# sikang/mpl_ros

Hardware: AMD Instinct MI355X
Metric: node_expansions_per_s (higher is better)
Workload: dtype f64

## Files before the change

include/mplx.h:

```cpp
#ifndef MPLX_H
#define MPLX_H
#include <stdint.h>

#ifdef __cplusplus
extern "C" {
#endif

#define MPLX_OK 0
#define MPLX_ERR_HIP (-1)
#define MPLX_ERR_ARG (-2)
#define MPLX_ERR_CAPACITY (-3)
#define MPLX_ERR_TIMEOUT (-4)

#define MPLX_PLAN_OK 0
#define MPLX_PLAN_NO_PATH 1
#define MPLX_PLAN_START_OCCUPIED 2
#define MPLX_PLAN_MAX_EXPAND 3
#define MPLX_PLAN_POOL_FULL 4
#define MPLX_PLAN_INTERNAL 5
#define MPLX_PLAN_TRAJ_TOO_LONG 6
#define MPLX_PLAN_ABORTED 7

#define MPLX_VEL 1
#define MPLX_ACC 3
// ... 226 lines not shown
int mplx_plpa_result_entries(mplx_plpa *l, uint64_t cap, int32_t *child, int32_t *parent, int32_t *action, int32_t *blocked);
typedef struct mplx_plpa_fleet mplx_plpa_fleet;
int mplx_plpa_fleet_create(mplx_poly *p, int32_t n, const int32_t *world_of, mplx_plpa_fleet **out);
void mplx_plpa_fleet_destroy(mplx_plpa_fleet *f);
const char *mplx_plpa_fleet_last_error(const mplx_plpa_fleet *f);
int mplx_plpa_fleet_size(const mplx_plpa_fleet *f);
mplx_plpa *mplx_plpa_fleet_member(mplx_plpa_fleet *f, int32_t i);
int mplx_plpa_fleet_set_capacity(mplx_plpa_fleet *f, uint64_t nodes, uint64_t edges, uint64_t open_log);
int mplx_plpa_fleet_set_world(mplx_plpa_fleet *f, int32_t i, int32_t world);
int mplx_plpa_fleet_plan(mplx_plpa_fleet *f, const double *starts, const double *goals, const int32_t *active, double eps, double tol_pos, double tol_vel,
                         int32_t max_expand, int32_t heur_ignore_dynamics, mplx_result *out);
int mplx_plpa_fleet_update_nodes(mplx_plpa_fleet *f, uint64_t *n_blocked, uint64_t *n_cleared);
int mplx_plpa_fleet_sub_state_space(mplx_plpa_fleet *f, const int32_t *time_step);
int mplx_plpa_fleet_stats(const mplx_plpa_fleet *f, uint32_t stats[4]);
int mplx_plpa_fleet_last_kernel_ms(const mplx_plpa_fleet *f, float *plan_ms, float *update_ms);
int mplx_poly_last_helpers(const mplx_poly *p);
int mplx_poly_set_deadline(mplx_poly *p, double seconds);
int mplx_poly_result_cycles(mplx_poly *p, int32_t q, uint64_t cyc[10]);

int mplx_result_timing(mplx_ctx *ctx, int q, double *t_begin_s, double *t_end_s, int32_t *slot);
int mplx_result_cycles(mplx_ctx *ctx, int q, uint64_t cyc[10]);
int mplx_result_speculation(mplx_ctx *ctx, int q, uint64_t spec[4]);
int mplx_result_open_dropped(mplx_ctx *ctx, int q, uint64_t *n_dropped);
int mplx_last_kernel_ms(const mplx_ctx *ctx, float *ms);
const char *mplx_kernel_name(const mplx_ctx *ctx);
uint64_t mplx_plan_epoch(const mplx_ctx *ctx);
const char *mplx_version(void);

typedef struct mplx_cloud mplx_cloud;
typedef struct {
  double state[13];
  double cost;
  int32_t action;
  int32_t valid;
} mplx_cloud_succ;
int mplx_cloud_create(int device, mplx_cloud **out);
void mplx_cloud_destroy(mplx_cloud *c);
const char *mplx_cloud_last_error(const mplx_cloud *c);
int mplx_cloud_config(mplx_cloud *c, int32_t control, int32_t n_u, const double *U, double dt, double v_max, double a_max, double j_max, double w);
int mplx_cloud_set_map(mplx_cloud *c, int32_t n, const double *pts, double r, const double ori[3], const double dim[3]);
int mplx_cloud_get_succ_batch(mplx_cloud *c, int32_t K, const double *states, mplx_cloud_succ *out);
uint64_t mplx_cloud_last_point_tests(const mplx_cloud *c);
int mplx_cloud_set_capacity(mplx_cloud *c, int32_t n_slots, uint64_t total_nodes, uint64_t total_edges, uint64_t total_open_log);
int mplx_cloud_plan_batch(mplx_cloud *c, int32_t n, const double *starts, const double *goals, double eps, double tol_pos, double tol_vel,
                          double tol_acc, int32_t max_expand, int32_t heur_ignore_dynamics, mplx_result *out);
int mplx_cloud_result_traj(mplx_cloud *c, int32_t q, mplx_waypoint *wps, int32_t *actions, int32_t *node_ids);
// ... 43 lines not shown
```

mpl_ros_amd/_capi.py:

```python
import ctypes as C
import os

_HERE = os.path.dirname(os.path.abspath(__file__))
LIB_PATH = os.environ.get("MPLX_LIB") or os.path.join(_HERE, "csrc", "libmplx.so")

VEL, ACC, JRK, SNP = 1, 3, 7, 15
PLAN_OK, PLAN_NO_PATH, PLAN_START_OCCUPIED, PLAN_MAX_EXPAND, PLAN_POOL_FULL, PLAN_INTERNAL, PLAN_TRAJ_TOO_LONG = 0, 1, 2, 3, 4, 5, 6
OK, ERR_HIP, ERR_ARG, ERR_CAPACITY, ERR_TIMEOUT = 0, -1, -2, -3, -4


class Waypoint(C.Structure):
    _fields_ = [("pos", C.c_double * 3), ("vel", C.c_double * 3), ("acc", C.c_double * 3),
                ("jrk", C.c_double * 3), ("yaw", C.c_double), ("t", C.c_double),
                ("control", C.c_int32), ("enable_t", C.c_int32)]


class Primitive(C.Structure):
    _fields_ = [("c", (C.c_double * 6) * 3), ("t", C.c_double), ("control", C.c_int32), ("pad", C.c_int32),
                ("cyaw", C.c_double * 6)]


class Config(C.Structure):
    _fields_ = [("control", C.c_int32), ("n_u", C.c_int32), ("U", C.POINTER(C.c_double)),
                ("dt", C.c_double), ("v_max", C.c_double), ("a_max", C.c_double), ("j_max", C.c_double),
# ... 8 lines not shown
                ("key", C.c_int32 * 12), ("nkey", C.c_int32), ("voxel_reads", C.c_int32)]


class Result(C.Structure):
    _fields_ = [("status", C.c_int32), ("traj_len", C.c_int32), ("cost", C.c_double)] + \
               [(n, C.c_uint64) for n in ("n_expanded", "n_closed", "n_nodes", "n_edges", "n_primitives", "n_succ",
                                          "n_succ_finite", "voxel_reads", "n_push", "n_reopen", "n_refill", "n_evict",
                                          "expand_hash")]

    def as_dict(self):
        return {n: getattr(self, n) for n, _ in self._fields_}


class CloudSucc(C.Structure):
    _fields_ = [("state", C.c_double * 13), ("cost", C.c_double), ("action", C.c_int32), ("valid", C.c_int32)]


EXPORTS = [
    "mplx_ctx_create", "mplx_ctx_destroy", "mplx_last_error", "mplx_set_stream",
    "mplx_map_set", "mplx_map_set_device", "mplx_map_free_unknown", "mplx_map_get", "mplx_map_info", "mplx_map_query",
    "mplx_map_dilate", "mplx_map_cells", "mplx_map_raytrace", "mplx_map_cloud",
    "mplx_planner_config", "mplx_set_capacity", "mplx_set_bucket_width", "mplx_set_speculation", "mplx_set_helpers", "mplx_helper_stats",
    "mplx_expand_batch", "mplx_heuristic_batch", "mplx_plan", "mplx_plan_batch",
    "mplx_result_traj", "mplx_set_record", "mplx_result_expanded", "mplx_result_nodes", "mplx_result_edges", "mplx_result_blocked", "mplx_result_timing", "mplx_result_cycles", "mplx_result_speculation", "mplx_result_open_dropped",
    "mplx_last_kernel_ms", "mplx_version", "mplx_kernel_name", "mplx_plan_epoch",
    "mplx_grid_create", "mplx_grid_destroy", "mplx_grid_last_error", "mplx_grid_allocate", "mplx_grid_info", "mplx_grid_clear",
    "mplx_grid_add_cloud", "mplx_grid_add_cloud_inflate", "mplx_grid_decay", "mplx_grid_clear_column", "mplx_grid_fill_column",
    "mplx_grid_fill_cell", "mplx_grid_get_map", "mplx_grid_get_cloud", "mplx_grid_to_map",
    "mplx_potential_weights", "mplx_potential_update", "mplx_search_region_set", "mplx_potential_clear", "mplx_aux_get", "mplx_aux_cloud", "mplx_aux_token",
    "mplx_lpa_create", "mplx_lpa_destroy", "mplx_lpa_last_error", "mplx_lpa_set_capacity", "mplx_lpa_set_record", "mplx_lpa_plan", "mplx_lpa_initialized",
    "mplx_lpa_reset", "mplx_lpa_update_blocked", "mplx_lpa_update_cleared", "mplx_lpa_sub_state_space", "mplx_lpa_set_reroot", "mplx_lpa_traj_len", "mplx_lpa_result_traj",
    "mplx_lpa_counts", "mplx_lpa_result_nodes", "mplx_lpa_result_edges", "mplx_lpa_result_expanded", "mplx_lpa_last_kernel_ms",
    "mplx_lpa_fleet_create", "mplx_lpa_fleet_destroy", "mplx_lpa_fleet_last_error", "mplx_lpa_fleet_size", "mplx_lpa_fleet_member", "mplx_lpa_fleet_set_capacity",
    "mplx_lpa_fleet_plan", "mplx_lpa_fleet_update_blocked", "mplx_lpa_fleet_update_cleared", "mplx_lpa_fleet_sub_state_space", "mplx_lpa_fleet_stats",
    "mplx_lpa_fleet_last_kernel_ms",
    "mplx_poly_create", "mplx_poly_destroy", "mplx_poly_last_error", "mplx_poly_config", "mplx_poly_begin", "mplx_poly_set_world",
    "mplx_poly_add_static", "mplx_poly_add_linear", "mplx_poly_add_nonlinear", "mplx_poly_commit", "mplx_poly_get_succ_batch", "mplx_poly_set_capacity", "mplx_poly_plan_batch", "mplx_poly_result_traj",
    "mplx_poly_set_record", "mplx_poly_result_expanded", "mplx_poly_last_kernel_ms", "mplx_poly_result_cycles", "mplx_poly_set_helpers", "mplx_poly_last_helpers", "mplx_poly_set_deadline", "mplx_plpa_create", "mplx_plpa_destroy", "mplx_plpa_last_error", "mplx_plpa_set_capacity", "mplx_plpa_initialized", "mplx_plpa_reset",
    "mplx_plpa_plan", "mplx_plpa_update_nodes", "mplx_plpa_changed", "mplx_plpa_sub_state_space", "mplx_plpa_traj_len", "mplx_plpa_result_traj", "mplx_plpa_last_kernel_ms", "mplx_plpa_result_cycles",
    "mplx_plpa_counts", "mplx_plpa_result_expanded", "mplx_plpa_result_nodes", "mplx_plpa_result_entries",
    "mplx_plpa_fleet_create", "mplx_plpa_fleet_destroy", "mplx_plpa_fleet_last_error", "mplx_plpa_fleet_size", "mplx_plpa_fleet_member", "mplx_plpa_fleet_set_capacity",
    "mplx_plpa_fleet_set_world", "mplx_plpa_fleet_plan", "mplx_plpa_fleet_update_nodes", "mplx_plpa_fleet_sub_state_space", "mplx_plpa_fleet_stats",
    "mplx_plpa_fleet_last_kernel_ms",
    "mplx_traj_solve", "mplx_traj_sample", "mplx_traj_effort",
    "mplx_plan_batch_submit", "mplx_plan_batch_wait", "mplx_plan_batch_done", "mplx_set_helper_limit", "mplx_release_pools",
    "mplx_set_deadline", "mplx_set_pool_recycling", "mplx_debug_hang_next_launch", "mplx_debug_query_records",
    "mplx_stream_create", "mplx_stream_destroy", "mplx_stream_last_error", "mplx_stream_depth", "mplx_stream_configure",
# ... 49 lines not shown
    L.mplx_map_cells.argtypes = [P, C.c_int, C.c_void_p, C.c_void_p]
    L.mplx_map_raytrace.argtypes = [P, D3, D3, C.c_void_p, C.c_int, C.POINTER(C.c_int)]
    L.mplx_map_cloud.argtypes = [P, C.c_int, C.c_void_p, C.c_uint64, C.POINTER(C.c_uint64)]
    L.mplx_planner_config.argtypes = [P, C.POINTER(Config)]
    L.mplx_set_capacity.argtypes = [P, C.c_int32, C.c_uint64, C.c_uint64, C.c_uint64]
    L.mplx_set_bucket_width.argtypes = [P, C.c_double]
    L.mplx_set_speculation.argtypes = [P, C.c_int32]
    L.mplx_set_helpers.argtypes = [P, C.c_int32, C.c_int32, C.c_uint64]
    L.mplx_helper_stats.argtypes = [P, C.POINTER(C.c_uint32)]
    L.mplx_expand_batch.argtypes = [P, C.c_int, C.POINTER(Waypoint), C.POINTER(Succ)]
    L.mplx_heuristic_batch.argtypes = [P, C.c_int, C.POINTER(Waypoint), C.POINTER(Waypoint), C.c_void_p, C.c_void_p]
    L.mplx_plan.argtypes = [P, C.POINTER(Waypoint), C.POINTER(Waypoint), C.POINTER(Result)]
    L.mplx_plan_batch.argtypes = [P, C.c_int, C.POINTER(Waypoint), C.POINTER(Waypoint), C.POINTER(Result)]
    L.mplx_result_traj.argtypes = [P, C.c_int, C.POINTER(Primitive), C.POINTER(Waypoint), I3, I3]
    L.mplx_set_record.argtypes = [P, C.c_uint32]
    L.mplx_result_expanded.argtypes = [P, C.c_int, C.c_uint32, C.c_void_p, C.POINTER(C.c_uint32)]
    L.mplx_result_nodes.argtypes = [P, C.c_uint64, C.POINTER(Waypoint), C.c_void_p, C.c_void_p, C.c_void_p, C.c_void_p]
    L.mplx_result_edges.argtypes = [P, C.c_void_p, C.c_void_p, C.c_void_p, C.c_uint64, C.POINTER(C.c_uint64)]
    L.mplx_result_blocked.argtypes = [P, C.c_void_p, C.c_void_p, C.c_uint64, C.POINTER(C.c_uint64), C.POINTER(C.c_uint64)]
    L.mplx_result_timing.argtypes = [P, C.c_int, C.POINTER(C.c_double), C.POINTER(C.c_double), I3]
    L.mplx_result_cycles.argtypes = [P, C.c_int, C.POINTER(C.c_uint64)]
    L.mplx_result_speculation.argtypes = [P, C.c_int, C.POINTER(C.c_uint64)]
    L.mplx_result_open_dropped.argtypes = [P, C.c_int, C.POINTER(C.c_uint64)]
    L.mplx_last_kernel_ms.argtypes = [P, C.POINTER(C.c_float)]
    L.mplx_version.restype = C.c_char_p
    L.mplx_kernel_name.argtypes = [P]
    L.mplx_kernel_name.restype = C.c_char_p
    L.mplx_plan_epoch.argtypes = [P]
    L.mplx_plan_epoch.restype = C.c_uint64
    L.mplx_traj_solve.argtypes = [C.c_int32, C.c_int32, C.POINTER(Waypoint), D3, C.POINTER(Primitive)]
    L.mplx_traj_sample.argtypes = [C.c_int32, C.POINTER(Primitive), C.c_int32, C.POINTER(Waypoint), C.c_void_p]
    L.mplx_traj_effort.argtypes = [C.c_int32, C.POINTER(Primitive), C.c_int32]
    L.mplx_traj_effort.restype = C.c_double
    U64 = C.POINTER(C.c_uint64)
    L.mplx_potential_weights.argtypes = [P, C.c_double, C.c_double]
    L.mplx_potential_update.argtypes = [P, D3, D3, D3, C.c_int32]
    L.mplx_search_region_set.argtypes = [P, C.c_int, C.c_void_p, D3, C.c_int]
    L.mplx_potential_clear.argtypes = [P]
    L.mplx_aux_get.argtypes = [P, C.c_void_p]
    L.mplx_aux_token.argtypes = [P, C.c_uint64, C.c_int32, U64]
    L.mplx_aux_cloud.argtypes = [P, C.c_int, C.c_void_p, C.c_void_p, C.c_uint64, U64]
    L.mplx_lpa_create.argtypes = [P, C.POINTER(P)]
    L.mplx_lpa_destroy.argtypes = [P]
    L.mplx_lpa_destroy.restype = None
    L.mplx_lpa_last_error.argtypes = [P]
    L.mplx_lpa_last_error.restype = C.c_char_p
# ... 171 lines not shown
```

mpl_ros_amd/csrc/mplx_api.hip:

```cpp
#include "../../include/mplx.h"

#include <hip/hip_runtime.h>

#include <sched.h>
#include <unistd.h>

#include <algorithm>
#include <chrono>
#include <cmath>
#include <cstdarg>
#include <cstdio>
#include <cstring>
#include <string>
#include <vector>

#define MPLX_UTILITY_KERNELS
#include "mplx_kernels.h"
#include "mplx_poly_dev.h"

using namespace mplx;

static_assert(sizeof(SuccOut) == sizeof(mplx_succ), "SuccOut must mirror mplx_succ");
static_assert(sizeof(State) == 12 * sizeof(double), "State layout");

static std::string g_create_error;

struct mplx_ctx {
  int device = 0;
  hipStream_t stream = nullptr;
  bool own_stream = true;
  std::string err;
  int8_t *map = nullptr;
  bool own_map = false;
  uint32_t *bricks = nullptr;
  int8_t *aux = nullptr;
  double pot_weight = 0.0;
  uint64_t aux_token = 0;
  int32_t dim[3] = {0, 0, 0};
  double origin[3] = {0, 0, 0};
  double res = 0;
// ... 11 lines not shown
  int helpers = -1;
  int help_reserved = -1;
  uint64_t help_rows = 0;
  int n_cus = 0;
  int pool_help_lanes = 0;
  int32_t n_slots = 1;
  uint64_t cap_nodes = 1u << 20, cap_edges = 1u << 22, cap_log = 1u << 21;
  uint32_t cap_rec = 0;
  bool pools_valid = false;
  int32_t pool_slots = 0, pool_control = 0;
  uint64_t pool_nodes = 0, pool_edges = 0, pool_log = 0;
  SearchParams pools{};
  std::vector<void *> pool_allocs;
  std::vector<uint32_t> last_node_table;
  int last_nq = 0;
  bool last_single = false;
  int last_control = 0;
  double last_dt = 0;
  std::vector<double> last_U;
  uint64_t plan_epoch = 0;
  bool help_cache_filled = false;
  uint64_t map_epoch = 0, last_map_epoch = 0;
  std::vector<QueryOut> last_out;
  QueryOut *d_out = nullptr;
  QueryIn *d_in = nullptr;
  int32_t *d_traj_nodes = nullptr, *d_traj_actions = nullptr, *d_rec = nullptr, *d_next = nullptr, *d_order = nullptr;
  uint32_t *d_node_tables = nullptr, *d_edge_tables = nullptr;
  double *d_traj_states = nullptr;
  int batch_cap = 0;
  uint32_t batch_rec = 0;
  hipEvent_t ev0 = nullptr, ev1 = nullptr;
  float last_ms = 0;
  uint32_t help_epoch = 0;
  unsigned long long help_done_init = 0;
  HelpBox *dbg_boxes = nullptr;
  uint32_t help_stats[4] = {0, 0, 0, 0};
  uint32_t help_ctr_back[HELP_CTR_WORDS] = {};
  bool help_stats_pending = false;
  bool pending = false;
  int pend_nq = 0;
  bool pend_help = false;
  std::vector<QueryIn> pend_in;
  std::vector<int32_t> pend_order;
  bool recycle = false;
  uint32_t *d_chunk_bits = nullptr;
  std::vector<uint32_t> chunk_bits_init;
// ... 875 lines not shown
    uint32_t *ctr = nullptr;
    PA(ctr, HELP_CTR_WORDS);
    P.cache_next = ctr;
    P.done_word = (unsigned long long *)(ctr + 32);
    P.cache_rows = (uint32_t)rows;
  }
#undef PA
  P.node_chunks = (uint32_t)nch;
  P.edge_chunks = (uint32_t)ech;
  P.open_chunks = (uint32_t)och;
  P.table_mask = T - 1;
  c->pool_slots = slots;
  c->pool_control = control;
  c->pool_nodes = c->cap_nodes;
  c->pool_edges = c->cap_edges;
  c->pool_log = c->cap_log;
  c->pools_valid = true;
  return MPLX_OK;
}

static int ensure_batch(mplx_ctx *c, int nq) {
  if (c->batch_cap >= nq && c->batch_rec == c->cap_rec) return MPLX_OK;
  free_batch(c);
  HIPCHK(c, hipMalloc((void **)&c->d_out, sizeof(QueryOut) * nq));
  HIPCHK(c, hipMalloc((void **)&c->d_in, sizeof(QueryIn) * nq));
  HIPCHK(c, hipMalloc((void **)&c->d_traj_nodes, sizeof(int32_t) * (size_t)nq * (MAX_TRAJ + 1)));
  HIPCHK(c, hipMalloc((void **)&c->d_traj_actions, sizeof(int32_t) * (size_t)nq * MAX_TRAJ));
  HIPCHK(c, hipMalloc((void **)&c->d_traj_states, sizeof(double) * (size_t)nq * (MAX_TRAJ + 1) * 13));
  HIPCHK(c, hipMalloc((void **)&c->d_traj_yaw, sizeof(double) * (size_t)nq * (MAX_TRAJ + 1)));
  HIPCHK(c, hipMalloc((void **)&c->d_next, sizeof(int32_t)));
  HIPCHK(c, hipMalloc((void **)&c->d_order, sizeof(int32_t) * nq));
  HIPCHK(c, hipMalloc((void **)&c->d_node_tables, sizeof(uint32_t) * (size_t)nq * MAX_NODE_CH));
  HIPCHK(c, hipMalloc((void **)&c->d_edge_tables, sizeof(uint32_t) * (size_t)nq * MAX_EDGE_CH));
  if (c->cap_rec) HIPCHK(c, hipMalloc((void **)&c->d_rec, sizeof(int32_t) * (size_t)nq * c->cap_rec));
  c->batch_cap = nq;
  c->batch_rec = c->cap_rec;
  return MPLX_OK;
}

static void wp_to_state(const mplx_waypoint &w, State &s) {
  for (int i = 0; i < 3; i++) {
    s.p[i] = w.pos[i];
    s.v[i] = (w.control & 2) ? w.vel[i] : 0.0;
    s.a[i] = (w.control & 4) ? w.acc[i] : 0.0;
    s.j[i] = (w.control & 8) ? w.jrk[i] : 0.0;
  }
}
// ... 180 lines not shown
  }
  SearchParams P = c->pools;
  fill_params(c, P, (c->speculation < 0 || c->speculation > 1) && (c->cfg.control == CTRL_ACC || c->cfg.control == CTRL_JRK) && c->cfg.n_u <= 128);
  if (c->wedged) return fail(c, MPLX_ERR_TIMEOUT, "this context was lost to a launch that never ended (destroy it)");
  const int xflags = getenv("MPLX_X_FLAGS") ? atoi(getenv("MPLX_X_FLAGS")) : 0;
  P.xflags = xflags | (c->debug_hang ? 8 : 0);
  c->debug_hang = false;
  guard_arm(c);
  P.cap_rec = c->cap_rec;
  P.nq = nq;
  P.queries = c->d_in;
  P.order = c->d_order;
  P.out = c->d_out;
  P.traj_nodes = c->d_traj_nodes; P.traj_actions = c->d_traj_actions; P.traj_states = c->d_traj_states;
  P.traj_yaw = c->d_traj_yaw;
  P.rec_ids = c->cap_rec ? c->d_rec : nullptr;
  P.node_tables = c->d_node_tables;
  P.edge_tables = c->d_edge_tables;
  P.next_query = c->d_next;
  if (c->filter_table) filter_set(P, c->filter_table, c->filter_mask, c->filter_pool, c->filter_flag);
  HIPCHK(c, hipMemcpyAsync(c->d_order, order.data(), sizeof(int32_t) * nq, hipMemcpyHostToDevice, c->stream));
  if (int rt = table_prepare(c, P, c->stream)) return rt;
  HIPCHK(c, hipMemsetAsync(P.chunk_next, 0, 4 * sizeof(uint32_t), c->stream));
  P.chunk_bits = nullptr;
  HIPCHK(c, hipMemcpyAsync(c->d_in, in.data(), sizeof(QueryIn) * nq, hipMemcpyHostToDevice, c->stream));
  HIPCHK(c, hipMemsetAsync(c->d_next, 0, sizeof(int32_t), c->stream));
  const bool spec = (c->speculation < 0 || c->speculation > 1) && !c->yaw;
  const bool recycle = c->recycle && nq > 1 && spec && !c->filter_table && (P.control == CTRL_ACC || P.control == CTRL_JRK) && P.n_u <= 128 && c->d_chunk_bits;
  if (recycle) {
    HIPCHK(c, hipMemcpyAsync(c->d_chunk_bits, c->chunk_bits_init.data(), sizeof(uint32_t) * c->chunk_bits_init.size(), hipMemcpyHostToDevice, c->stream));
    P.chunk_bits = c->d_chunk_bits;
    for (int k = 0; k < 3; k++) { P.chunk_word0[k] = c->chunk_word0[k]; P.chunk_words[k] = c->chunk_words[k]; }
  }
  c->last_recycled = recycle;
  const int n_wg = c->n_cus;
  int grid = slots;
  P.help_lead = slots;
  P.help_max = 0;
  P.help_limit = c->help_limit;
  const bool help = spec && !c->aux && !c->filter_table && (c->speculation < 0 || c->speculation >= 16) && c->helpers != 0 && P.boxes &&
                    ((P.n_u <= 31 && (P.control == CTRL_ACC || P.control == CTRL_JRK)) || (P.control == CTRL_JRK && P.n_u > 64 && P.n_u <= 128));
  if (help) {
    P.help_max = c->helpers < 0 ? (P.n_u <= 31 ? 4 : 2) : c->helpers;
    P.help_lead = std::min(slots, n_wg);
    const bool long_queries = P.max_expand <= 0 || P.max_expand >= 200000;
    const int reserved = c->help_reserved >= 0 ? c->help_reserved : (nq >= 2 * c->n_cus && long_queries ? std::max(1, c->n_cus / 16) * P.help_max : 0);
// ... 48 lines not shown
}

static int plan_batch_finish(mplx_ctx *c, mplx_result *out) {
  if (!c->pending) return fail(c, MPLX_ERR_ARG, "no submitted batch on this context");
  HIPCHK(c, hipSetDevice(c->device));
  const int nq = c->pend_nq;
  c->pending = false;
  {
    const int rw = guard_wait(c, c->stream, "the search launch");
    if (rw) {
      c->last_nq = 0;
      return rw;
    }
  }
  if (c->pend_help) {
    HIPCHK(c, hipMemcpyAsync(c->help_ctr_back, c->pools.cache_next, HELP_CTR_WORDS * sizeof(uint32_t), hipMemcpyDeviceToHost, c->stream));
    c->help_stats_pending = true;
  } else {
    memset(c->help_stats, 0, sizeof(c->help_stats));
    c->help_stats_pending = false;
  }
  c->last_out.resize(nq);
  HIPCHK(c, hipMemcpyAsync(c->last_out.data(), c->d_out, sizeof(QueryOut) * nq, hipMemcpyDeviceToHost, c->stream));
  HIPCHK(c, hipStreamSynchronize(c->stream));
  HIPCHK(c, hipEventElapsedTime(&c->last_ms, c->ev0, c->ev1));
  if (out)
    for (int i = 0; i < nq; i++) fill_result(c->last_out[i], out[i]);
  c->last_nq = nq;
  c->last_single = (nq == 1);
  c->last_control = c->cfg.control;
  c->last_dt = c->cfg.dt;
  c->last_U = c->U;
  c->last_yaw = c->yaw;
  c->last_Uyaw = c->Uyaw;
  c->last_map_epoch = c->map_epoch;
  c->plan_epoch++;
  return MPLX_OK;
}

extern "C" int mplx_plan_batch(mplx_ctx *c, int nq, const mplx_waypoint *starts, const mplx_waypoint *goals, mplx_result *out) {
  if (!out) return fail(c, MPLX_ERR_ARG, "bad argument");
  int r = plan_batch_launch(c, nq, starts, goals);
  if (r) return r;
  return plan_batch_finish(c, out);
}

// ... 458 lines not shown
  if (t_end_s) *t_end_s = (double)(c->last_out[q].t_end - t0) * 1e-8;
  if (slot) *slot = (int32_t)c->last_out[q].slot;
  return MPLX_OK;
}

extern "C" int mplx_result_cycles(mplx_ctx *c, int q, uint64_t cyc[10]) {
  if (!c || q < 0 || q >= c->last_nq || !cyc) return fail(c, MPLX_ERR_ARG, "no such query");
  for (int i = 0; i < 10; i++) cyc[i] = c->last_out[q].cyc[i];
  return MPLX_OK;
}

extern "C" int mplx_result_speculation(mplx_ctx *c, int q, uint64_t spec[4]) {
  if (!c || q < 0 || q >= c->last_nq || !spec) return fail(c, MPLX_ERR_ARG, "no such query");
  for (int i = 0; i < 4; i++) spec[i] = c->last_out[q].spec[i];
  return MPLX_OK;
}

extern "C" int mplx_result_open_dropped(mplx_ctx *c, int q, uint64_t *n_dropped) {
  if (!c || q < 0 || q >= c->last_nq || !n_dropped) return fail(c, MPLX_ERR_ARG, "no such query");
  *n_dropped = query_open_dropped(c->last_out[q]);
  return MPLX_OK;
}

extern "C" int mplx_last_kernel_ms(const mplx_ctx *c, float *ms) {
  if (!c || !ms) return MPLX_ERR_ARG;
  *ms = c->last_ms;
  return MPLX_OK;
}
#include "mplx_lpa.inl"
#include "mplx_lpa_fleet.inl"
#include "mplx_grid.inl"
#include "mplx_poly_search.h"
#include "mplx_poly.inl"
#include "mplx_ctx_ext.inl"
```

mpl_ros_amd/csrc/mplx_help_launch.hip:

```cpp
#include <hip/hip_runtime.h>

#include "mplx_spec.h"

using namespace mplx;

bool mplx_launch_spec_help(int grid, hipStream_t s, const SearchParams &P) {
  if (!(P.control == CTRL_ACC || P.control == CTRL_JRK) || !P.boxes) return false;
#ifdef MPLX_ONLY_ACC
  if (P.control != CTRL_ACC || P.n_u > 31) return false;
  hipLaunchKernelGGL((astar_spec_kernel<32, 16, CTRL_ACC, 1024, 1024, true>), dim3(grid), dim3(512), 0, s, P);
  return true;
#else
  if (P.control == CTRL_JRK && P.n_u > 64 && P.n_u <= 128) {
    hipLaunchKernelGGL((astar_spec_kernel<128, 4, CTRL_JRK, 1024, 1024, true>), dim3(grid), dim3(512), 0, s, P);
    return true;
  }
  if (P.n_u > 31) return false;
  if (P.control == CTRL_ACC)
    hipLaunchKernelGGL((astar_spec_kernel<32, 16, CTRL_ACC, 1024, 1024, true>), dim3(grid), dim3(512), 0, s, P);
  else
    hipLaunchKernelGGL((astar_spec_kernel<32, 16, CTRL_JRK, 1024, 1024, true>), dim3(grid), dim3(512), 0, s, P);
  return true;
#endif
}
```

mpl_ros_amd/csrc/mplx_spec.h:

```cpp
#pragma once
#include "mplx_kernels.h"

#ifdef MPLX_LOOKUP_TIMERS
#define MPLX_T2(S, k, var) do { if (threadIdx.x == 0) { const unsigned long long now_ = __builtin_readcyclecounter(); (S).cyc2[k] += now_ - (var); var = now_; } } while (0)
#else
#define MPLX_T2(S, k, var) do { } while (0)
#endif

#ifndef MPLX_X_LDS_CONST
#define MPLX_X_LDS_CONST 1
#endif
#ifndef MPLX_X_EARLY_SETUP
#define MPLX_X_EARLY_SETUP 1
#endif
#ifndef MPLX_X_EARLY_ROW
#define MPLX_X_EARLY_ROW 1
#endif
#ifndef MPLX_X_EARLY_TOMB
#define MPLX_X_EARLY_TOMB 0
#endif
#ifndef MPLX_X_ROW_FENCE
#define MPLX_X_ROW_FENCE 0
#endif
#define MPLX_ROW_FENCE(P) (MPLX_X_ROW_FENCE || MPLX_XF(P, 16))
#define MPLX_EARLY_TOMB(P) (MPLX_X_EARLY_TOMB || MPLX_XF(P, 32))
#ifndef MPLX_X_EARLY_CLEAR
#define MPLX_X_EARLY_CLEAR 1
#endif
#ifndef MPLX_X_PROBE2
#define MPLX_X_PROBE2 1
#endif

namespace mplx {

__device__ __forceinline__ void lds_barrier() {
  __builtin_amdgcn_fence(__ATOMIC_RELEASE, "workgroup", "local");
  __builtin_amdgcn_s_barrier();
  __builtin_amdgcn_fence(__ATOMIC_ACQUIRE, "workgroup", "local");
}

template <int UL, int K, int CONTROL, int BTN, int NCAP_, bool YAW = false>
struct SmemSpec : Smem<UL * K, K, NCAP_> {
  static constexpr int BLOCK = UL * K, BT = BTN, NK = key_len_c(CONTROL) + (YAW ? 1 : 0);
  static_assert(NK <= MAX_KEY, "yaw-carrying SNP states (13 key integers) stay on the one-node kernel");
  double cand_f[K], cand_g[K];
  uint32_t cand_id[K], cand_idx[K], cand_pos[K];
  int32_t cand_live[K];
  uint32_t cand_fl[K];
  int32_t n_cand;
  uint32_t u_succ[K], u_fin[K], u_reads[K];
  int32_t unit_seq[K];
  uint32_t cur_slot[K];
  unsigned long long bt_hash[BT];
// ... 13 lines not shown
  uint32_t app_id[256], app_rank[256];
  uint32_t csum[2][UL * K / 64];
  int32_t batch_dep;
  int32_t any_shared;
  int32_t dep_cause;
  int32_t cut_at;
  int32_t helped;
  unsigned long long box_seq;
  int32_t help_box, help_idx, help_q, help_go, help_quit;
#ifdef MPLX_HELP_DEBUG
  unsigned long long dbg_t, dbg_gap, dbg_when;
#endif
  unsigned long long help_seq;
  int32_t help_idle;
  uint32_t n_work;
  uint32_t work[WISH];
  unsigned long long wish_l[WISH];
#ifdef MPLX_LOOKUP_TIMERS
  unsigned long long cyc2[24];
  unsigned long long cycw[16][4];
  unsigned long long arr_max, arr_heur, sum_heur, sum_arr;
  unsigned long long dbg_n, dbg_na, dbg_slow, dbg_n256, dbg_pulls;
#endif
};

struct LanePre {
  double tg, pf;
  int code;
  int cut;
};

template <int UL, int K, int CONTROL, bool PAR, bool HELP, bool YAW, class SM, class V>
__device__ __forceinline__ void spec_commit_lanes(const V &Q, SM &S, int tid, int q, int kc, bool active, int my_slot, int k_stop,
                                                  const LaneSucc &L, double hspec, const LanePre &pre, uint32_t &pend_idx, uint32_t &pend_old, int par = 0) {
  constexpr int BLOCK = UL * K;
  constexpr int nk = key_len_c(CONTROL), ns = key_len_c(CONTROL);
  const SearchParams &P = Q.P;
  const int lu = tid % UL;
  const bool isnew = active && S.bt_id[my_slot] == NIL;
  if (active && pend_idx != NIL) {
    Q.open(pend_idx)->next = pend_old;
    pend_idx = NIL;
  }
  double old_g = INFINITY, tg = 0.0;
  uint32_t fl = 0, old_pred = NIL, id = NIL;
  bool improved = false;
// ... 350 lines not shown
          } else {
            atomicAnd(&B->helpers, ~(1u << S.help_idx));
            S.help_box = -1;
          }
        }
      }
    }
    __syncthreads();
    if (S.help_box < 0) {
      if (tid == 0) S.help_idle++;
      for (int i = 0; i < 16; i++) __builtin_amdgcn_s_sleep(127);
      __syncthreads();
      continue;
    }
    helper_serve<UL, K, CONTROL>(P, S, tid);
    if (tid == 0) {
      atomicAnd(&(P.boxes + S.help_box)->helpers, ~(1u << S.help_idx));
      S.help_idle = 0;
    }
    __syncthreads();
  }
}

template <int UL, int K, int CONTROL, int BTN, int NCAP_, bool HELP = false, bool POT = false, bool YAW = false, bool FILTER = false>
__global__ __launch_bounds__(UL *K) void astar_spec_kernel(SearchParams P) {
  static_assert(!(FILTER && (HELP || POT || YAW)), "the filtered search is the plain kernel");
  static_assert(!(HELP && POT), "the look-ahead cache rows carry no potential sums");
  static_assert(!(YAW && (HELP || POT)), "yaw-carrying searches run without helpers and without an auxiliary map");
  constexpr int BLOCK = UL * K;
  using SM = SmemSpec<UL, K, CONTROL, BTN, NCAP_, YAW>;
  constexpr int BT = SM::BT;
  __shared__ SM S;
  using V = QView<BLOCK, CONTROL, SM>;
  const int tid = threadIdx.x, ku = tid / UL, lu = tid % UL;
  const V Q{P, S, P.bkt_head + (size_t)blockIdx.x * 2 * NB * NSUB};
  constexpr int nk = key_len_c(CONTROL), ns = key_len_c(CONTROL);
  constexpr int NKY = nk + (YAW ? 1 : 0), EX = YAW ? 1 : 0;
  constexpr bool DROP = !(HELP && CONTROL == CTRL_JRK && UL == 128);
  auto lane_hash = [&](const LaneSucc &l) {
    if constexpr (YAW) {
      int32_t kk[MAX_KEY + 1];
#pragma unroll
      for (int i = 0; i < nk; i++) kk[i] = l.key[i];
      kk[nk] = l.yaw_key;
      return key_hash64(kk, NKY);
    } else {
      return key_hash64(l.key, nk);
    }
  };
  auto goal_reached = [&](const State &s, double yaw) {
    bool g = is_goal_state(s, S.hp.goal, S.hp.goal_control & 15, P.tol_pos, P.tol_vel, P.tol_acc);
    if (YAW && g && P.tol_yaw >= 0) g = fabs(yaw - S.hp.goal_yaw) <= P.tol_yaw;
    return g;
  };
  auto ld_state = [&](const double *p) -> double {
    if constexpr (HELP) {
      if (!MPLX_XF(P, 128)) return ld_f64_agent(p);
    }
    return *p;
  };
  fill_uq<BLOCK, CONTROL>(P, S, tid);
// ... 9 lines not shown
    if (tid == 0) {
      if (HELP && (int)blockIdx.x >= P.help_lead) S.q_index = P.nq;
      else {
        S.q_index = atomicAdd(P.next_query, 1);
        if (guard_abort(P)) S.q_index = P.nq;
      }
    }
    __syncthreads();
    const int qi = S.q_index;
    if (qi >= P.nq) break;
    const int q = P.order[qi];
    const QueryIn &in = P.queries[q];
    const unsigned long long t_begin = wall_clock64();
    query_reset(Q, in, (uint32_t)(K * P.n_u + K), tid);
    if (tid == 0) {
      S.n_sorted = 0;
#ifdef MPLX_LOOKUP_TIMERS
      for (int i = 0; i < 24; i++) S.cyc2[i] = 0;
      for (int i = 0; i < 64; i++) (&S.cycw[0][0])[i] = 0;
      S.arr_max = 0; S.arr_heur = 0; S.sum_heur = 0; S.sum_arr = 0;
      S.dbg_n = S.dbg_na = S.dbg_slow = S.dbg_n256 = S.dbg_pulls = 0;
#endif
      S.c_cand = S.c_live = S.c_cut = S.c_drop = 0;
      S.cur_id = NIL;
      S.helped = 0;
      S.box_seq = 0;
      if constexpr (HELP) {
        HelpBox *box = P.boxes + blockIdx.x;
        st_u32(&box->q, (uint32_t)q);
        st_u32(&box->rank, (uint32_t)qi);
#ifdef MPLX_HELP_DEBUG
        box->xcc_plus1 = dbg_xcc() + 1u;
        S.dbg_t = wall_clock64();
        S.dbg_gap = 0;
        S.dbg_when = 0;
#endif
        st_u64(&box->n_expanded, 0ull);
        st_u64(&box->seq, ((unsigned long long)P.epoch << 32) | 1ull);
      }
      query_admit(Q, in, voxel_start_free(P, in), goal_reached(in.start, in.start_yaw));
    }
    __syncthreads();
    bool searched = false;
    if (S.status < 0) {
      searched = true;
      const int32_t ykey = (int32_t)round(in.start_yaw / KEY_RES_YAW);
// ... 67 lines not shown
        }
        MPLX_TIC(tp);
        [[maybe_unused]] unsigned long long t3 = __builtin_readcyclecounter();
        batch_no++;
        if (S.n_near == 0) {
          __syncthreads();
          if (!refill<BLOCK, CONTROL, SM, DROP>(Q, tid)) {
            if (tid == 0) S.status = 1;
            __syncthreads();
            break;
          }
          if (tid == 0) S.n_sorted = 0;
          __syncthreads();
        }
        const unsigned long long evict0 = S.c_evict;
        for (int guard = 0; guard < 8 && S.n_near < (uint32_t)K; guard++) {
          __syncthreads();
          const uint32_t before = S.n_near;
          if (!refill<BLOCK, CONTROL, SM, DROP>(Q, tid)) break;
          if (tid == 0 && S.c_evict != evict0) S.n_sorted = 0;
          (void)before;
          __syncthreads();
        }
        MPLX_T2(S, 16, t3);
#if MPLX_X_EARLY_SETUP
#ifdef MPLX_HELP_DEBUG
        if (HELP && tid == 0) {
          HelpBox *box = P.boxes + blockIdx.x;
          const unsigned long long now = wall_clock64(), gap = now - S.dbg_t;
          S.dbg_t = now;
          if (gap > S.dbg_gap) { S.dbg_gap = gap; S.dbg_when = ((now - t_begin) << 1) | (S.helped ? 1ull : 0ull); }
          if (gap > 1000000ull) {
            if (gap > box->pad1[0]) { box->pad1[0] = gap; box->pad1[1] = S.dbg_when; box->pad1[2] = (unsigned long long)q; box->pad1[3] = S.cyc[7]; }
          }
        }
#endif
        MPLX_T2(S, 17, t3);
#else
        if (tid == 0) {
          S.cyc[7]++;
          S.n_cand = 0;
          S.cut_at = K;
          S.batch_dep = 0;
          S.any_shared = 0;
          S.dep_cause = 0;
          if constexpr (HELP) {
// ... 265 lines not shown
              pos = (pos + 1) & (size_t)F.mask;
            }
            if (!ok) S.cand_live[opaque(ku)] = 0;
          }
          unit_sync<UL>();
          live_unit = live_unit && S.cand_live[opaque(ku)] != 0;
        }
        if (live_unit && lu == 0) {
          State sgoal;
          for (int i = 0; i < 12; i++) ((double *)&sgoal)[i] = S.cur[ku][i];
#if MPLX_X_LDS_CONST
          S.u_goal[ku] = (S.cur[ku][12] >= P.t_max || goal_reached(sgoal, YAW ? S.cur_yaw[ku] : 0.0)) ? 1 : 0;
#else
          S.u_goal[ku] = (S.cur[ku][12] >= P.t_max || goal_reached(sgoal, YAW ? S.cur_yaw[ku] : 0.0)) ? 1 : 0;
#endif
        }
        if constexpr (HELP) {
          if (live_unit && S.helped && !MPLX_XF(P, 256) && lu == UL - 1 && (uint32_t)hc_a != 0u && ((uint32_t)hc_b & CACHE_READY) &&
              (uint32_t)(hc_a >> 32) == (uint32_t)key_hash64(S.cur_key[ku], nk)) {
            S.hc_row[ku] = (uint32_t)hc_a;
            S.hc_valid[ku] = (uint32_t)hc_b;
            S.hc_blocked[ku] = (uint32_t)(hc_b >> 32);
            atomicAdd(&S.cyc[9], 1ull);
          }
        }
        unit_sync<UL>();
        [[maybe_unused]] double h_row = 0.0;
        [[maybe_unused]] unsigned long long reads_word = 0ull;
        [[maybe_unused]] unsigned long long h_tag = 0ull, reads_tag = 0ull;
        [[maybe_unused]] uint32_t reads_row = 0u;
#if MPLX_X_EARLY_ROW
        if constexpr (HELP) {
          const uint32_t rp1 = live_unit ? S.hc_row[ku] : 0u;
          if MPLX_XF(P, 2) __builtin_amdgcn_fence(__ATOMIC_ACQUIRE, "agent");
          if (rp1) {
            const double *row = P.cache_h + (size_t)(rp1 - 1u) * cache_row_doubles(UL);
            bool want = lu < P.n_u && P.eps != 0.0;
            if constexpr (UL <= 64) want = want && (((S.hc_valid[ku] & ~S.hc_blocked[ku]) >> lu) & 1u);
            if (want) h_row = ld_f64_agent(&row[cache_h_slot(UL, lu)]);
#if MPLX_X_ROW_PAIRS
            if constexpr (UL == 32) {
              if (want) h_tag = ld_u64((const unsigned long long *)&row[cache_h_slot(UL, lu) + 1]);
              if (lu == 0) reads_tag = ld_u64((const unsigned long long *)&row[cache_reads_slot(UL) + 1]);
            }
#endif
            if (lu == 0) {
// ... 456 lines not shown
            const uint32_t pos = S.n_near + (uint32_t)__popcll(mb & below);
            S.near_f[pos] = S.cand_f[l]; S.near_g[pos] = S.cand_g[l]; S.near_id[pos] = cur; S.near_idx[pos] = S.cand_idx[l];
          }
          static_assert(K <= 16, "exponents up to 16: S.hpow");
          const unsigned long long term = row_incl_sum64(done ? (unsigned long long)(cur + 1u) * S.hpow[__popcll((m >> l) >> 1) & 31] : 0ull);
          const unsigned long long terms = ((unsigned long long)(uint32_t)__builtin_amdgcn_readlane((int)(uint32_t)(term >> 32), 15) << 32) |
                                           (unsigned long long)(uint32_t)__builtin_amdgcn_readlane((int)(uint32_t)term, 15);
          const unsigned long long hh = S.c_hash * S.hpow[__popcll(m) & 31] + terms;
          if (m && l == 63 - __clzll((long long)m)) S.cur_id = cur;
          if (l == 0) {
            const unsigned long long ncm = (unsigned long long)__popcll(m);
            S.c_expanded = ne0 + ncm;
            S.c_closed += ncm;
            S.c_hash = hh;
            S.c_prims += ncm * (unsigned long long)P.n_u;
            S.c_succ += su;
            S.c_succ_finite += fi;
            S.c_reads += rd;
            S.n_near += (uint32_t)__popcll(mb);
            S.c_cand += (unsigned long long)n_cand;
            S.c_live += (unsigned long long)__popcll(live_m);
            S.c_cut += (unsigned long long)__popcll(mb);
            if (!parallel_commit) S.cyc[8]++;
          }
        }
#if MPLX_X_EARLY_SETUP
        batch_setup(S.c_expanded);
#endif
        __syncthreads();
        MPLX_T2(S, 13, t2);
        MPLX_TOC(S, 6, to);
        if (S.status >= 0) break;
      }
    }
    const uint32_t goal_id = searched ? S.cur_id : NIL;
    if (searched) clear_buckets(Q, tid);
    if constexpr (HELP) {
      if (tid == 0) st_u64(&(P.boxes + blockIdx.x)->seq, (unsigned long long)P.epoch << 32);
    }
    __syncthreads();
    if (tid == 0) {
      query_report<EX>(Q, q, goal_id, [&](uint32_t, uint32_t action) {
        return (POT && P.map.aux) ? P.ucost[action & EDGE_ACTION_MASK] + P.pot_weight * (double)(action >> EDGE_POT_SHIFT) : P.ucost[action & EDGE_ACTION_MASK];
      }, SpecCounts{{S.c_cand, S.c_cand - S.c_live, S.c_live, S.c_cut}}, t_begin, ld_state);
      P.out[q].n_refill |= (unsigned long long)S.c_drop << 32;
#ifdef MPLX_LOOKUP_TIMERS
      if (P.nq == 1 || q % 61 == 0) {
      printf("cyc2 q%d batches %llu:", q, S.cyc[7]);
      for (int i = 0; i < 24; i++) printf(" %llu", S.cyc2[i] / (S.cyc[7] ? S.cyc[7] : 1ull));
      printf("\n  max-over-lanes: heuristic done %llu, barrier arrival %llu\n", S.sum_heur / S.cyc[7], S.sum_arr / S.cyc[7]);
      printf("  ranking: mean near size %.1f, mean appended %.1f, batches on the all-pairs path %llu, batches with near > 256: %llu, of %llu\n", (double)S.dbg_n / S.cyc[7], (double)S.dbg_na / S.cyc[7], S.dbg_slow, S.dbg_n256, S.cyc[7]);
      for (int j = 0; j < 4; j++) { printf("  per-wave %d:", j); for (int w = 0; w < BLOCK / 64; w++) printf(" %llu", S.cycw[w][j] / (S.cyc[7] ? S.cyc[7] : 1ull)); printf("\n"); }
      }
#endif
    }
    bool recycled = false;
    if (P.chunk_bits) {
      recycled = true;
      if constexpr (HELP) {
        if (P.boxes) {
          if (tid == 0) {
            int ok = 1;
            const HelpBox *box = P.boxes + blockIdx.x;
            for (uint32_t polls = 0; ld_u32(&box->helpers) != 0u; polls++) {
              if (polls > 40000u || ((polls & 1023u) == 1023u && guard_abort(P))) { ok = 0; break; }
              __builtin_amdgcn_s_sleep(32);
            }
            S.flag = ok;
// ... 46 lines not shown
```

mpl_ros_amd/planner.py:

```python
import ctypes as C
import sys
import weakref
import math

import numpy as np

from . import _capi
from ._capi import ACC, JRK, SNP, VEL, MplxError


class Control:
    VEL, ACC, JRK, SNP = VEL, ACC, JRK, SNP


class Waypoint3D:

    def __init__(self, control=0):
        self.pos = np.zeros(3)
        self.vel = np.zeros(3)
        self.acc = np.zeros(3)
        self.jrk = np.zeros(3)
        self.yaw = 0.0
        self.t = 0.0
        self.enable_t = False
# ... 688 lines not shown
        ctx = self._ctx()
        b, e, s = C.c_double(), C.c_double(), C.c_int32()
        ctx.check(ctx.lib.mplx_result_timing(ctx.h, q, C.byref(b), C.byref(e), C.byref(s)))
        return b.value, e.value, s.value

    def queryCycles(self, q=0):
        ctx = self._ctx()
        cyc = (C.c_uint64 * 10)()
        ctx.check(ctx.lib.mplx_result_cycles(ctx.h, q, cyc))
        return dict(zip(("pop", "expand", "lookup", "evict", "refill", "activate", "commit", "batches", "dep_batches", "cache_hits"), [int(x) for x in cyc[:10]]))

    def querySpeculation(self, q=0):
        ctx = self._ctx()
        sp = (C.c_uint64 * 4)()
        ctx.check(ctx.lib.mplx_result_speculation(ctx.h, q, sp))
        return dict(zip(("candidates", "stale", "units_expanded", "units_cut"), [int(x) for x in sp[:4]]))

    def queryOpenDropped(self, q=0):
        ctx = self._ctx()
        n = C.c_uint64(0)
        ctx.check(ctx.lib.mplx_result_open_dropped(ctx.h, q, C.byref(n)))
        return int(n.value)

    def getTrajCost(self):
        return self.traj_cost_

    def getResult(self, q=0):
        return self._results[q]

    def getTraj(self, q=0):
        ctx = self._own_results()
        res = self._results[q]
        n = res.traj_len if res.status == _capi.PLAN_OK else 0
        if self._use_lpastar and self._lpa is not None:
            n = int(ctx.lib.mplx_lpa_traj_len(self._lpa.h))
        if n <= 0:
            return Trajectory3D([], [], np.zeros(0, dtype=np.int32), res.cost)
        prs = (_capi.Primitive * n)()
        wps = (_capi.Waypoint * (n + 1))()
        act = (C.c_int32 * n)()
        ids = (C.c_int32 * (n + 1))()
        if self._use_lpastar and self._lpa is not None:
            self._lpa.check(ctx.lib.mplx_lpa_result_traj(self._lpa.h, prs, wps, act, ids))
        else:
            ctx.check(ctx.lib.mplx_result_traj(ctx.h, q, prs, wps, act, ids))
        P = [Primitive3D([list(prs[i].c[k]) for k in range(3)], prs[i].t, prs[i].control, list(prs[i].cyaw)) for i in range(n)]
# ... 408 lines not shown
```

Measured before the change: 78.80 million.

## Refill open-list early when near buffer runs low during helped search

Adds an early refill step in the speculative A* kernel: when helpers are active and the near buffer holds fewer than K plus a lead margin while the next bucket run can supply at least K nodes, the kernel pulls from the bucket queue ahead of time. The goal is to keep enough candidates buffered so helper blocks and the main loop stall less waiting on refills. It also adds per-query counters for cache misses and early pulls, exported through a new API and extra output memory. The early refill adds barriers and may evict sorted prefixes, which could cost more than it saves.

```diff
diff --git a/include/mplx.h b/include/mplx.h
--- a/include/mplx.h
+++ b/include/mplx.h
@@ -272,6 +272,7 @@
 int mplx_result_cycles(mplx_ctx *ctx, int q, uint64_t cyc[10]);
 int mplx_result_speculation(mplx_ctx *ctx, int q, uint64_t spec[4]);
 int mplx_result_open_dropped(mplx_ctx *ctx, int q, uint64_t *n_dropped);
+int mplx_result_open_lead(mplx_ctx *ctx, int q, uint64_t lead[7]);
 int mplx_last_kernel_ms(const mplx_ctx *ctx, float *ms);
 const char *mplx_kernel_name(const mplx_ctx *ctx);
 uint64_t mplx_plan_epoch(const mplx_ctx *ctx);
diff --git a/mpl_ros_amd/_capi.py b/mpl_ros_amd/_capi.py
--- a/mpl_ros_amd/_capi.py
+++ b/mpl_ros_amd/_capi.py
@@ -54,7 +54,7 @@
     "mplx_map_dilate", "mplx_map_cells", "mplx_map_raytrace", "mplx_map_cloud",
     "mplx_planner_config", "mplx_set_capacity", "mplx_set_bucket_width", "mplx_set_speculation", "mplx_set_helpers", "mplx_helper_stats",
     "mplx_expand_batch", "mplx_heuristic_batch", "mplx_plan", "mplx_plan_batch",
-    "mplx_result_traj", "mplx_set_record", "mplx_result_expanded", "mplx_result_nodes", "mplx_result_edges", "mplx_result_blocked", "mplx_result_timing", "mplx_result_cycles", "mplx_result_speculation", "mplx_result_open_dropped",
+    "mplx_result_traj", "mplx_set_record", "mplx_result_expanded", "mplx_result_nodes", "mplx_result_edges", "mplx_result_blocked", "mplx_result_timing", "mplx_result_cycles", "mplx_result_speculation", "mplx_result_open_dropped", "mplx_result_open_lead",
     "mplx_last_kernel_ms", "mplx_version", "mplx_kernel_name", "mplx_plan_epoch",
     "mplx_grid_create", "mplx_grid_destroy", "mplx_grid_last_error", "mplx_grid_allocate", "mplx_grid_info", "mplx_grid_clear",
     "mplx_grid_add_cloud", "mplx_grid_add_cloud_inflate", "mplx_grid_decay", "mplx_grid_clear_column", "mplx_grid_fill_column",
@@ -150,6 +150,7 @@
     L.mplx_result_cycles.argtypes = [P, C.c_int, C.POINTER(C.c_uint64)]
     L.mplx_result_speculation.argtypes = [P, C.c_int, C.POINTER(C.c_uint64)]
     L.mplx_result_open_dropped.argtypes = [P, C.c_int, C.POINTER(C.c_uint64)]
+    L.mplx_result_open_lead.argtypes = [P, C.c_int, C.POINTER(C.c_uint64)]
     L.mplx_last_kernel_ms.argtypes = [P, C.POINTER(C.c_float)]
     L.mplx_version.restype = C.c_char_p
     L.mplx_kernel_name.argtypes = [P]
diff --git a/mpl_ros_amd/csrc/mplx_api.hip b/mpl_ros_amd/csrc/mplx_api.hip
--- a/mpl_ros_amd/csrc/mplx_api.hip
+++ b/mpl_ros_amd/csrc/mplx_api.hip
@@ -16,6 +16,7 @@
 
 #define MPLX_UTILITY_KERNELS
 #include "mplx_kernels.h"
+#include "mplx_lead.h"
 #include "mplx_poly_dev.h"
 
 using namespace mplx;
@@ -73,6 +74,7 @@
   bool help_cache_filled = false;
   uint64_t map_epoch = 0, last_map_epoch = 0;
   std::vector<QueryOut> last_out;
+  std::vector<unsigned long long> last_lead;
   QueryOut *d_out = nullptr;
   QueryIn *d_in = nullptr;
   int32_t *d_traj_nodes = nullptr, *d_traj_actions = nullptr, *d_rec = nullptr, *d_next = nullptr, *d_order = nullptr;
@@ -994,7 +996,7 @@
 static int ensure_batch(mplx_ctx *c, int nq) {
   if (c->batch_cap >= nq && c->batch_rec == c->cap_rec) return MPLX_OK;
   free_batch(c);
-  HIPCHK(c, hipMalloc((void **)&c->d_out, sizeof(QueryOut) * nq));
+  HIPCHK(c, hipMalloc((void **)&c->d_out, query_out_bytes(nq)));
   HIPCHK(c, hipMalloc((void **)&c->d_in, sizeof(QueryIn) * nq));
   HIPCHK(c, hipMalloc((void **)&c->d_traj_nodes, sizeof(int32_t) * (size_t)nq * (MAX_TRAJ + 1)));
   HIPCHK(c, hipMalloc((void **)&c->d_traj_actions, sizeof(int32_t) * (size_t)nq * MAX_TRAJ));
@@ -1221,6 +1223,7 @@
   HIPCHK(c, hipMemcpyAsync(c->d_order, order.data(), sizeof(int32_t) * nq, hipMemcpyHostToDevice, c->stream));
   if (int rt = table_prepare(c, P, c->stream)) return rt;
   HIPCHK(c, hipMemsetAsync(P.chunk_next, 0, 4 * sizeof(uint32_t), c->stream));
+  HIPCHK(c, hipMemsetAsync(query_lead_stats(c->d_out, nq, 0), 0, sizeof(unsigned long long) * LEAD_STATS * (size_t)nq, c->stream));
   P.chunk_bits = nullptr;
   HIPCHK(c, hipMemcpyAsync(c->d_in, in.data(), sizeof(QueryIn) * nq, hipMemcpyHostToDevice, c->stream));
   HIPCHK(c, hipMemsetAsync(c->d_next, 0, sizeof(int32_t), c->stream));
@@ -1315,6 +1318,8 @@
   }
   c->last_out.resize(nq);
   HIPCHK(c, hipMemcpyAsync(c->last_out.data(), c->d_out, sizeof(QueryOut) * nq, hipMemcpyDeviceToHost, c->stream));
+  c->last_lead.resize((size_t)LEAD_STATS * nq);
+  HIPCHK(c, hipMemcpyAsync(c->last_lead.data(), query_lead_stats(c->d_out, nq, 0), sizeof(unsigned long long) * LEAD_STATS * (size_t)nq, hipMemcpyDeviceToHost, c->stream));
   HIPCHK(c, hipStreamSynchronize(c->stream));
   HIPCHK(c, hipEventElapsedTime(&c->last_ms, c->ev0, c->ev1));
   if (out)
@@ -1819,6 +1824,14 @@
   return MPLX_OK;
 }
 
+extern "C" int mplx_result_open_lead(mplx_ctx *c, int q, uint64_t lead[7]) {
+  if (!c || q < 0 || q >= c->last_nq || !lead) return fail(c, MPLX_ERR_ARG, "no such query");
+  static_assert(LEAD_STATS == 7, "mplx.h");
+  const bool have = c->last_lead.size() == (size_t)LEAD_STATS * (size_t)c->last_nq;
+  for (int i = 0; i < LEAD_STATS; i++) lead[i] = have ? c->last_lead[(size_t)q * LEAD_STATS + i] : 0ull;
+  return MPLX_OK;
+}
+
 extern "C" int mplx_last_kernel_ms(const mplx_ctx *c, float *ms) {
   if (!c || !ms) return MPLX_ERR_ARG;
   *ms = c->last_ms;
diff --git a/mpl_ros_amd/csrc/mplx_help_acc_launch.hip b/mpl_ros_amd/csrc/mplx_help_acc_launch.hip
--- /dev/null
+++ b/mpl_ros_amd/csrc/mplx_help_acc_launch.hip
@@ -0,0 +1,9 @@
+#include <hip/hip_runtime.h>
+
+#include "mplx_spec.h"
+
+using namespace mplx;
+
+void mplx_launch_spec_help_acc(int grid, hipStream_t s, const SearchParams &P) {
+  hipLaunchKernelGGL((astar_spec_kernel<32, 16, CTRL_ACC, 1024, 1024, true>), dim3(grid), dim3(512), 0, s, P);
+}
diff --git a/mpl_ros_amd/csrc/mplx_help_launch.hip b/mpl_ros_amd/csrc/mplx_help_launch.hip
--- a/mpl_ros_amd/csrc/mplx_help_launch.hip
+++ b/mpl_ros_amd/csrc/mplx_help_launch.hip
@@ -4,11 +4,19 @@
 
 using namespace mplx;
 
+void mplx_launch_spec_help_acc(int grid, hipStream_t s, const SearchParams &P);
+
+#ifndef MPLX_ONLY_ACC
+void mplx_help_unit_companion(int grid, hipStream_t s, const SearchParams &P) {
+  hipLaunchKernelGGL((astar_spec_kernel<32, 16, CTRL_ACC, 1024, 512, true>), dim3(grid), dim3(512), 0, s, P);
+}
+#endif
+
 bool mplx_launch_spec_help(int grid, hipStream_t s, const SearchParams &P) {
   if (!(P.control == CTRL_ACC || P.control == CTRL_JRK) || !P.boxes) return false;
 #ifdef MPLX_ONLY_ACC
   if (P.control != CTRL_ACC || P.n_u > 31) return false;
-  hipLaunchKernelGGL((astar_spec_kernel<32, 16, CTRL_ACC, 1024, 1024, true>), dim3(grid), dim3(512), 0, s, P);
+  mplx_launch_spec_help_acc(grid, s, P);
   return true;
 #else
   if (P.control == CTRL_JRK && P.n_u > 64 && P.n_u <= 128) {
@@ -17,7 +25,7 @@
   }
   if (P.n_u > 31) return false;
   if (P.control == CTRL_ACC)
-    hipLaunchKernelGGL((astar_spec_kernel<32, 16, CTRL_ACC, 1024, 1024, true>), dim3(grid), dim3(512), 0, s, P);
+    mplx_launch_spec_help_acc(grid, s, P);
   else
     hipLaunchKernelGGL((astar_spec_kernel<32, 16, CTRL_JRK, 1024, 1024, true>), dim3(grid), dim3(512), 0, s, P);
   return true;
diff --git a/mpl_ros_amd/csrc/mplx_lead.h b/mpl_ros_amd/csrc/mplx_lead.h
--- /dev/null
+++ b/mpl_ros_amd/csrc/mplx_lead.h
@@ -0,0 +1,10 @@
+#pragma once
+#include "mplx_device.h"
+
+namespace mplx {
+constexpr int LEAD_STATS = 7;
+constexpr size_t query_out_bytes(int nq) { return (sizeof(QueryOut) + LEAD_STATS * sizeof(unsigned long long)) * (size_t)nq; }
+__host__ __device__ inline unsigned long long *query_lead_stats(QueryOut *out, int nq, int q) {
+  return (unsigned long long *)(out + nq) + (size_t)q * LEAD_STATS;
+}
+}
diff --git a/mpl_ros_amd/csrc/mplx_spec.h b/mpl_ros_amd/csrc/mplx_spec.h
--- a/mpl_ros_amd/csrc/mplx_spec.h
+++ b/mpl_ros_amd/csrc/mplx_spec.h
@@ -1,5 +1,6 @@
 #pragma once
 #include "mplx_kernels.h"
+#include "mplx_lead.h"
 
 #ifdef MPLX_LOOKUP_TIMERS
 #define MPLX_T2(S, k, var) do { if (threadIdx.x == 0) { const unsigned long long now_ = __builtin_readcyclecounter(); (S).cyc2[k] += now_ - (var); var = now_; } } while (0)
@@ -29,6 +30,10 @@
 #endif
 #ifndef MPLX_X_PROBE2
 #define MPLX_X_PROBE2 1
+#endif
+
+#ifndef MPLX_X_LEAD
+#define MPLX_X_LEAD 3
 #endif
 
 namespace mplx {
@@ -88,6 +93,7 @@
   unsigned long long arr_max, arr_heur, sum_heur, sum_arr;
   unsigned long long dbg_n, dbg_na, dbg_slow, dbg_n256, dbg_pulls;
 #endif
+  uint32_t since_pull, pulls_seen, c_miss[4], c_early, c_early_long, c_early_evict;
 };
 
 struct LanePre {
@@ -484,6 +490,21 @@
   }
 }
 
+template <int BLOCK, class SM>
+__device__ __forceinline__ uint32_t next_run_count(const SM &S, int lane) {
+  constexpr int MAXB = MPLX_X_MERGE_PULL && BLOCK >= NSUB ? MERGE_CUR * BLOCK / NSUB : 1;
+  const int b = (S.cur0 > 0 ? S.cur0 : 0) + lane;
+  const uint32_t c = b < NB ? S.cnt[0][b] : 0u;
+  const unsigned long long m = __ballot(c > 0u);
+  if (m == 0ull) return 0u;
+  const uint32_t pre = wave_incl_sum<64>(c);
+  const int first = __builtin_ctzll(m), rank = __popcll(m & ((1ull << lane) - 1ull));
+  const uint32_t used = S.n_near + S.reserve, cap = used < (uint32_t)SM::NCAP ? (uint32_t)SM::NCAP - used : 0u;
+  const uint32_t target = cap < (uint32_t)MERGE_TARGET ? cap : (uint32_t)MERGE_TARGET;
+  const unsigned long long tm = __ballot(c > 0u && (lane == first || (rank < MAXB && pre <= target)));
+  return (uint32_t)__builtin_amdgcn_readlane((int)pre, 63 - __clzll((long long)tm));
+}
+
 template <int UL, int K, int CONTROL, int BTN, int NCAP_, bool HELP = false, bool POT = false, bool YAW = false, bool FILTER = false>
 __global__ __launch_bounds__(UL *K) void astar_spec_kernel(SearchParams P) {
   static_assert(!(FILTER && (HELP || POT || YAW)), "the filtered search is the plain kernel");
@@ -499,6 +520,8 @@
   constexpr int nk = key_len_c(CONTROL), ns = key_len_c(CONTROL);
   constexpr int NKY = nk + (YAW ? 1 : 0), EX = YAW ? 1 : 0;
   constexpr bool DROP = !(HELP && CONTROL == CTRL_JRK && UL == 128);
+  constexpr int LEAD = DROP ? MPLX_X_LEAD * K : 0;
+  constexpr bool MISS_CTR = HELP && DROP;
   auto lane_hash = [&](const LaneSucc &l) {
     if constexpr (YAW) {
       int32_t kk[MAX_KEY + 1];
@@ -554,6 +577,10 @@
       S.dbg_n = S.dbg_na = S.dbg_slow = S.dbg_n256 = S.dbg_pulls = 0;
 #endif
       S.c_cand = S.c_live = S.c_cut = S.c_drop = 0;
+      if constexpr (LEAD > 0 || MISS_CTR) {
+        S.since_pull = S.pulls_seen = S.c_early = S.c_early_long = S.c_early_evict = 0;
+        S.c_miss[0] = S.c_miss[1] = S.c_miss[2] = S.c_miss[3] = 0;
+      }
       S.cur_id = NIL;
       S.helped = 0;
       S.box_seq = 0;
@@ -667,6 +694,23 @@
           (void)before;
           __syncthreads();
         }
+        if constexpr (LEAD > 0) {
+          if (((HELP && S.helped) || (P.xflags & 8192)) && S.n_near < (uint32_t)(K + LEAD) && next_run_count<BLOCK>(S, tid & 63) >= (uint32_t)K) {
+            __syncthreads();
+            const uint32_t prefix = S.n_sorted;
+            refill<BLOCK, CONTROL, SM, DROP>(Q, tid);
+            if (tid == 0) {
+              const bool evicted = S.c_evict != evict0;
+              if (evicted) S.n_sorted = 0;
+              S.c_early++;
+              if (prefix > (uint32_t)K) {
+                S.c_early_long++;
+                if (evicted) S.c_early_evict++;
+              }
+            }
+            __syncthreads();
+          }
+        }
         MPLX_T2(S, 16, t3);
 #if MPLX_X_EARLY_SETUP
 #ifdef MPLX_HELP_DEBUG
@@ -978,6 +1022,8 @@
             S.hc_valid[ku] = (uint32_t)hc_b;
             S.hc_blocked[ku] = (uint32_t)(hc_b >> 32);
             atomicAdd(&S.cyc[9], 1ull);
+          } else if (MISS_CTR && live_unit && S.helped && lu == UL - 1) {
+            atomicAdd(&S.c_miss[(uint32_t)S.c_refill != S.pulls_seen ? 0u : S.since_pull], 1u);
           }
         }
         unit_sync<UL>();
@@ -1480,6 +1526,11 @@
             S.c_live += (unsigned long long)__popcll(live_m);
             S.c_cut += (unsigned long long)__popcll(mb);
             if (!parallel_commit) S.cyc[8]++;
+            if constexpr (MISS_CTR) {
+              const uint32_t pulls = (uint32_t)S.c_refill, sp = pulls != S.pulls_seen ? 0u : S.since_pull;
+              S.since_pull = sp < 2u ? sp + 1u : 3u;
+              S.pulls_seen = pulls;
+            }
           }
         }
 #if MPLX_X_EARLY_SETUP
@@ -1502,6 +1553,13 @@
         return (POT && P.map.aux) ? P.ucost[action & EDGE_ACTION_MASK] + P.pot_weight * (double)(action >> EDGE_POT_SHIFT) : P.ucost[action & EDGE_ACTION_MASK];
       }, SpecCounts{{S.c_cand, S.c_cand - S.c_live, S.c_live, S.c_cut}}, t_begin, ld_state);
       P.out[q].n_refill |= (unsigned long long)S.c_drop << 32;
+      if constexpr (LEAD > 0 || MISS_CTR) {
+        unsigned long long *ls = query_lead_stats(P.out, P.nq, q);
+        for (int i = 0; i < 4; i++) ls[i] = S.c_miss[i];
+        ls[4] = S.c_early;
+        ls[5] = S.c_early_long;
+        ls[6] = S.c_early_evict;
+      }
 #ifdef MPLX_LOOKUP_TIMERS
       if (P.nq == 1 || q % 61 == 0) {
       printf("cyc2 q%d batches %llu:", q, S.cyc[7]);
diff --git a/mpl_ros_amd/planner.py b/mpl_ros_amd/planner.py
--- a/mpl_ros_amd/planner.py
+++ b/mpl_ros_amd/planner.py
@@ -734,6 +734,12 @@
         ctx.check(ctx.lib.mplx_result_open_dropped(ctx.h, q, C.byref(n)))
         return int(n.value)
 
+    def queryOpenLead(self, q=0):
+        ctx = self._ctx()
+        v = (C.c_uint64 * 7)()
+        ctx.check(ctx.lib.mplx_result_open_lead(ctx.h, q, v))
+        return dict(misses=[int(x) for x in v[:4]], early_pulls=int(v[4]), early_pulls_long_prefix=int(v[5]), early_pulls_evicting=int(v[6]))
+
     def getTrajCost(self):
         return self.traj_cost_
 
```

Result: faster. 81.65 million, median of 6 (+3.6%).
